# Scthe/cnn-Super-Resolution

Measured on AMD Instinct MI355X. Metric: training tiles/sec (fwd+bwd+update), default SRCNN 33x33, batch 4096/GPU, higher is better.
Workload: dtype f32

## Files before the change

### cnn-super-resolution_amd/csrc/hip/d1x6.hpp

```cpp

constexpr int kD6Mxx = 12, kD6Mx3 = 25;
constexpr int kD6ExWin = 6, kD6ExMid = 3;
constexpr int kD6Grow = 70;

constexpr int kD6Zero = 32;
__device__ __attribute__((aligned(16))) float g_d6_zero[kD6Zero] = {};
constexpr int d6_row_half(bool d3, int h) { return (d3 ? 4 : 8) * h; }
constexpr int d6_zero_half(bool d3, int h) { return d6_row_half(d3, h); }
constexpr int d6_row_quad(bool d3, int k) { return d3 ? 8 * k : 16 * (k >> 1) + 4 * (k & 1); }
constexpr bool d6_zero_row_covers(bool d3) {
  for (int h = 0; h < 2; h++)
    for (int k = 0; k < 4; k++)
      if (d6_zero_half(d3, h) + d6_row_quad(d3, k) + 4 > kD6Zero) return false;
  return true;
}

__device__ __forceinline__ void mma_x6_2(const bf16x8 (&a0)[3], const bf16x8 (&b0)[3], f32x16& c0,
                                         const bf16x8 (&a1)[3], const bf16x8 (&b1)[3], f32x16& c1) {
  using mfma::mma_bf16;
  c0 = mma_bf16(a0[2], b0[0], c0);
  c1 = mma_bf16(a1[2], b1[0], c1);
  c0 = mma_bf16(a0[1], b0[1], c0);
  c1 = mma_bf16(a1[1], b1[1], c1);
  c0 = mma_bf16(a0[0], b0[2], c0);
  c1 = mma_bf16(a1[0], b1[2], c1);
  c0 = mma_bf16(a0[1], b0[0], c0);
  c1 = mma_bf16(a1[1], b1[0], c1);
  c0 = mma_bf16(a0[0], b0[1], c0);
  c1 = mma_bf16(a1[0], b1[1], c1);
  c0 = mma_bf16(a0[0], b0[0], c0);
  c1 = mma_bf16(a1[0], b1[0], c1);
}

__device__ __forceinline__ void d6_split(const float (&v)[8], bf16x8 (&o)[3]) { mfma::split8(v, o); }

template <bool kD3, bool kTr = false>
__global__ __launch_bounds__(256, 1) void d1x6_grad12_kernel(const float* __restrict__ X,
                                                              const float* __restrict__ A1T,
                                                              const float* __restrict__ D2,
                                                              const float* __restrict__ A2,
                                                              const uint32_t* __restrict__ M2,
                                                              const float* __restrict__ W2,
                                                              const float* __restrict__ W3,
                                                              float* __restrict__ slab, Geom g, RunGeom rg,
                                                              D3Geom dg) {
  constexpr int N1 = 64, N2 = 32, F1 = 9, K1 = F1 * F1;
  constexpr int NW1 = K1 * N1, NW2 = N1 * N2, P12 = NW1 + N1 + NW2 + N2;
  extern __shared__ __attribute__((aligned(16))) float smem[];
  static_assert(kD3 || !kTr, "the part images belong to the delta3 form");
  const D6Lds L(g.W, g.H, rg, kD3);
  char* const base = reinterpret_cast<char*>(smem);
  __bf16* const w2i = reinterpret_cast<__bf16*>(base + L.w2);
  uint32_t* const u32 = reinterpret_cast<uint32_t*>(smem);
  uint32_t* const xbuf = u32 + L.xb / 4;
  int* const slots = reinterpret_cast<int*>(base + L.slots);
  int* const runs = reinterpret_cast<int*>(base + L.runs);

  SRCNN_CLOCK_BEGIN();
  const int lane = mfma::lane_id(), wave = mfma::wave_id();
  const int h = lane >> 5, li = lane & 31;
  const int W = g.W, xn = g.W * g.H, npx = g.ow * g.oh, nch = rg.nch;
  const int x0col = 4 * rg.a;

  float xr[kL12Regs];
  auto xload = [&](int smp) {
    const float* src = X + (size_t)smp * xn;
#pragma unroll
    for (int k = 0; k < kL12Regs; k++) {
      const int i = threadIdx.x + 256 * k;
      xr[k] = i < xn ? src[i] : 0.0f;
    }
  };
  if ((int)blockIdx.x < g.batch) xload(blockIdx.x);

  if constexpr (!kTr)
    for (int i = threadIdx.x; i < nch * 32; i += 256) slots[i] = slot_pixel(rg, i >> 5, i & 31);
  for (int k = threadIdx.x; k < nch * 8; k += 256) {
    int iy, ix;
    bool col;
    run_origin(rg, k < rg.nrun ? k : 0, iy, ix, col);
    runs[(k & ~7) + 4 * (k & 1) + 2 * ((k >> 2) & 1) + ((k >> 1) & 1)] =
        col ? ~(L.rdw + 3 * ((ix - x0col) * L.st + iy)) : 3 * (iy * L.rs + ix);
  }
  for (int i = threadIdx.x; i < (2 * L.xbuf + 3) / 4; i += 256) reinterpret_cast<uint4*>(xbuf)[i] = uint4{0u, 0u, 0u, 0u};
  if (threadIdx.x < 32 && (!kD3 || threadIdx.x < kD6Mxx || (threadIdx.x >= 16 && threadIdx.x < kD6Mx3)))
    u32[L.cst / 4 + threadIdx.x] = !kD3 && (threadIdx.x == 0 || threadIdx.x == 6) ? 0x3F803F80u : 0u;
  {
    constexpr int kIt = 2 * 2 * 64 * 8 / 256;
    float v[kIt];
#pragma unroll
    for (int k = 0; k < kIt; k++) {
      const int e = threadIdx.x + 256 * k;
      const int j = e & 7, L_ = (e >> 3) & 63, kk = (e >> 9) & 1, t = e >> 10;
      const int n = kD3 ? crow(8 * kk + j, L_ >> 5) : 16 * kk + 8 * (L_ >> 5) + j;
      v[k] = W2[(32 * t + (L_ & 31)) * N2 + n];
    }
#pragma unroll
    for (int k = 0; k < kIt; k++) {
      const int e = threadIdx.x + 256 * k;
      const int j = e & 7, L_ = (e >> 3) & 63, kk = (e >> 9) & 1, t = e >> 10;
      __bf16 p[3];
      split3(v[k], p[0], p[1], p[2]);
#pragma unroll
      for (int q = 0; q < 3; q++) w2i[((t * 2 + kk) * 3 + q) * 512 + L_ * 8 + j] = p[q];
    }
  }

  uint32_t* const d3u = u32 + L.d3img / 4;
  const int nout3 = dg.w3 * dg.h3;
// ... 21 lines not shown
          b16[2 * (d + L.gw * q) - 1] = b;
        }
      }
    }
  };
  float* const mxx = smem + L.cst / 4 + kD6Mxx;
  float* const mx3 = smem + L.cst / 4 + kD6Mx3;
  auto wave_max = [&](float v) {
#pragma unroll
    for (int o = 32; o > 0; o >>= 1) v = fmaxf(v, __shfl_xor(v, o, 64));
    return v;
  };
  auto put_max = [&](float* slot, float v) {
    v = wave_max(v);
    if (lane == 0) slot[wave] = v;
  };
  auto take_max_reg = [&](float v) {
    return __builtin_bit_cast(float, __builtin_amdgcn_readfirstlane(__builtin_bit_cast(int, v)));
  };
  auto take_max = [&](const float* slot) {
    const float v = fmaxf(fmaxf(slot[0], slot[1]), fmaxf(slot[2], slot[3]));
    return __builtin_bit_cast(float, __builtin_amdgcn_readfirstlane(__builtin_bit_cast(int, v)));
  };
  float m3cur = 0.0f, wnorm = 0.0f;
  int EW = 0, EB = 0, EWmin = 1 << 20, EBmin = 1 << 20;
  if constexpr (kD3) {
    {
      float n2 = 0.0f, n3 = 0.0f;
      for (int n = 0; n < N2; n++) n2 += fabsf(W2[lane * N2 + n]);
      for (int t = 0; t < dg.f3 * dg.f3; t++) n3 += fabsf(W3[t * N2 + li]);
      wnorm = take_max_reg(wave_max(n2)) * take_max_reg(wave_max(n3));
    }
    __bf16* const w3i = reinterpret_cast<__bf16*>(base + L.w3i);
    constexpr int kW3It = 2 * 64 * 8 / 256;
    static_assert(kW3It * 256 * 3 == kD6W3, "the W3 image: 2 k-steps x 3 parts");
    float w3v[kW3It];
#pragma unroll
    for (int k = 0; k < kW3It; k++) {
      const int e = threadIdx.x + 256 * k;
      const int j = e & 7, L_ = (e >> 3) & 63, s_ = e >> 9;
      const D3Pair tp = d3_pair_slot(8 * s_ + 4 * (L_ >> 5) + (j >> 1), dg.f3);
      const int dx = d3_pair_dx(tp, j & 1, dg.f3), n = L_ & 31;
      const bool in = dx >= 0;
      w3v[k] = W3[in ? (tp.dy * dg.f3 + dx) * N2 + n : 0];
      if (!in) w3v[k] = 0.0f;
    }
#pragma unroll
    for (int k = 0; k < kW3It; k++) {
      const int e = threadIdx.x + 256 * k;
      const int j = e & 7, L_ = (e >> 3) & 63, s_ = e >> 9;
      __bf16 p[3];
      split3(w3v[k], p[0], p[1], p[2]);
#pragma unroll
      for (int q = 0; q < 3; q++) w3i[((s_ * 3 + q) * 64 + L_) * 8 + j] = p[q];
    }
    int* const d3tab = reinterpret_cast<int*>(base + L.d3tab);
    for (int i = threadIdx.x; i < nch * 32; i += 256) {
      int iy, ix;
      slot_coord(rg, i >> 5, i & 31, iy, ix);
      d3tab[i] = kTr ? d6_slot_pack(slot_pixel(rg, i >> 5, i & 31), iy * L.gs + ix) : iy * L.gs + ix;
    }
    for (int i = threadIdx.x; i < (3 * L.d3buf + 3) / 4; i += 256)
      reinterpret_cast<uint4*>(d3u)[i] = uint4{0u, 0u, 0u, 0u};
    if ((int)blockIdx.x < g.batch) d3load(blockIdx.x);
    put_max(mx3, fmaxf(fabsf(d3n[0]), fabsf(d3n[1])));
    __syncthreads();
    m3cur = take_max(mx3);
    d3build(0);
    if ((int)blockIdx.x + (int)gridDim.x < g.batch) d3load(blockIdx.x + gridDim.x);
  }

  int offR3[3], offT3[3];
#pragma unroll
  for (int u = 0; u < 3; u++) {
    const int tap = 32 * u + li;
    const int dy = tap < K1 ? tap / F1 : 0, dx = tap < K1 ? tap - dy * F1 : 0;
    offR3[u] = 12 * (dy * L.rs + dx);
    offT3[u] = 12 * (dx * L.st + dy);
  }
  typedef __attribute__((address_space(3))) const uint32_t lds_u32;
  const int lds0 = (int)(uintptr_t)(__attribute__((address_space(3))) char*)base;
  const int spec = li == K1 - 64 ? lds0 + L.cst : li > K1 - 64 ? lds0 + L.cst + 64 : -1;

  f32x16 g1[2][3], g2[2];
#pragma unroll
  for (int t = 0; t < 2; t++) {
    g2[t] = zero16();
#pragma unroll
    for (int u = 0; u < 3; u++) g1[t][u] = zero16();
  }
// ... 179 lines not shown
    } else {
      take_rows();
    }
  }
  if constexpr (kTr) {
    sum_d2(1.0f);
#pragma unroll
    for (int k = 0; k < 2; k++) {
      split_d2(1 + k);
      tr_write(k);
    }
    __builtin_amdgcn_wave_barrier();
    tr_read(0);
    tr_read(1);
  } else {
    stage_d2();
#pragma unroll
    for (int piece = 0; piece < 5; piece++) split_d2(piece);
  }

  for (int it = 0; (int)blockIdx.x + it * (int)gridDim.x < g.batch; it++) {
    const int smp = blockIdx.x + it * gridDim.x;
    uint32_t* const xi = xbuf + (it & 1) * L.xbuf;
    float s1 = 1.0f, sX = 1.0f;
    float m3next = 0.0f;
    if constexpr (kD3) {
      float xm = 0.0f;
#pragma unroll
      for (int k = 0; k < kL12Regs; k++) xm = fmaxf(xm, fabsf(xr[k]));
      float dm = fmaxf(fabsf(d3n[0]), fabsf(d3n[1]));
#pragma unroll
      for (int o = 32; o > 0; o >>= 1) {
        const float tx = __shfl_xor(xm, o, 64), td = __shfl_xor(dm, o, 64);
        xm = fmaxf(xm, tx);
        dm = fmaxf(dm, td);
      }
      if (lane == 0) {
        mxx[wave] = xm;
        mx3[wave] = dm;
      }
      if (smp + (int)gridDim.x < g.batch) d3build((it + 1) - 3 * ((it + 1) / 3));
      __syncthreads();
      const float xmax = take_max(mxx);
      m3next = take_max(mx3);
      const float bound = m3cur * wnorm;
      int e1 = mfma::scale_exp_h(bound), exn = mfma::scale_exp_h(xmax), ex = 0, kb = 0, dW = 0, dB = 0;
      if (exn < mfma::kScaleMin + kD6ExMid) exn = mfma::kScaleMin + kD6ExMid;
      if (bound > 0.0f) {
        int exc = e1 + exn - kD6ExMid - (EWmin + kD6Grow);
        if (exc < e1 - (EBmin + kD6Grow)) exc = e1 - (EBmin + kD6Grow);
        if (exc > 0) e1 = e1 - exc < mfma::kScaleMin ? mfma::kScaleMin : e1 - exc;
        kb = EB - e1;
        if (kb < -14 || kb > 15) {
          dB = e1 - EB;
          EB = e1;
          kb = 0;
        }
        if (xmax > 0.0f) {
          ex = EW - e1;
          if (ex > exn || ex < exn - kD6ExWin) {
            ex = exn - kD6ExMid;
            dW = e1 + ex - EW;
            EW = e1 + ex;
          }
        }
        if (EW < EWmin) EWmin = EW;
        if (EB < EBmin) EBmin = EB;
      } else {
        e1 = 0;
        ex = xmax > 0.0f ? exn - kD6ExMid : 0;
      }
      s1 = mfma::pow2_h(e1);
      sX = mfma::pow2_h(ex);
      if (threadIdx.x == 0) {
        const uint32_t c = (uint32_t)(kb + 15) << 10;
        u32[L.cst / 4 + 3 * (it & 1)] = u32[L.cst / 4 + 3 * (it & 1) + 6] = c | (c << 16);
      }
      while (dW != 0 || dB != 0) {
        const int a = dW < -120 ? -120 : dW > 120 ? 120 : dW, b = dB < -120 ? -120 : dB > 120 ? 120 : dB;
        const float fw = mfma::pow2_h(a), fb = li == K1 - 64 ? mfma::pow2_h(b) : fw;
#pragma unroll
        for (int t = 0; t < 2; t++)
#pragma unroll
          for (int u = 0; u < 3; u++) {
            const float f = u == 2 ? fb : fw;
#pragma unroll
            for (int r = 0; r < 16; r++) g1[t][u][r] *= f;
            __builtin_amdgcn_sched_barrier(0);
          }
        dW -= a;
        dB -= b;
      }
    }
    if constexpr (kD3) {
      uint16_t* const x16 = reinterpret_cast<uint16_t*>(xi);
#pragma unroll
      for (int k = 0; k < kL12Regs; k++) {
        const int i = threadIdx.x + 256 * k;
        if (i < xn) {
          const float xs = xr[k] * sX;
          const _Float16 p0 = (_Float16)xs;
          const _Float16 p[2] = {p0, (_Float16)(xs - (float)p0)};
          const int y = i / W, x = i - y * W, ri = y * L.rs + x;
          const int ti = L.rdw + 3 * ((x - x0col) * L.st + y);
#pragma unroll
          for (int q = 0; q < 2; q++) {
            const uint16_t b = __builtin_bit_cast(uint16_t, p[q]);
            x16[2 * (3 * ri + q)] = b;
            if (ri > 0) x16[2 * (3 * (ri - 1) + q) + 1] = b;
            if (L.tcols && x >= x0col) {
              x16[2 * (ti + q)] = b;
              if (y > 0) x16[2 * (ti - 3 + q) + 1] = b;
            }
          }
        }
// ... 226 lines not shown
            }
            stage_d2();
          }
          if (st == 1) split_d2(0);
          if (st >= 1 && st <= 4) split_d2(st);
        } else if (st < 2) {
          split_d1(1, st);
          if (st == 1) split_d2(0);
        } else {
          split_d2(st - 1);
        }
#pragma unroll
        for (int i = 0; i < (kD3 ? 6 : 12); i++) {
          __builtin_amdgcn_sched_group_barrier(0x008, 1, 0);
          __builtin_amdgcn_sched_group_barrier(0x002, kD3 ? 12 : 6, 0);
          __builtin_amdgcn_sched_group_barrier(0x100, kD3 ? 2 : 1, 0);
        }
        __builtin_amdgcn_sched_barrier(0);
      }
      ki += 4;
      kj = nj;
      kc = nc;
    }
    m3cur = m3next;
  }
  SRCNN_CLOCK_END(g_clk, 2);

  __syncthreads();
  float* const red = smem;
  float* out = slab + (size_t)blockIdx.x * P12;
  float* const stg = smem + 4 * 4 * 16 * 64;
  auto stg_w1 = [&](int row, int ch) -> float& { return stg[row * N1 + (ch ^ ((row & 15) << 2))]; };
  auto tile_ref = [&](int k) -> f32x16& { return k < 6 ? g1[k / 3][k % 3] : g2[k - 6]; };
#pragma unroll
  for (int rd = 0; rd < 2; rd++) {
#pragma unroll
    for (int k = 0; k < 4; k++) {
      const f32x16& a = tile_ref(4 * rd + k);
#pragma unroll
      for (int r = 0; r < 16; r++) red[((k * 4 + wave) * 16 + r) * 64 + lane] = a[r];
    }
    __syncthreads();
#pragma unroll
    for (int k = 0; k < 4; k++) {
      if (wave != k) continue;
      const int tile = 4 * rd + k;
      f32x16 sum;
// ... 62 lines not shown
```

### cnn-super-resolution_amd/csrc/hip/fused_layout.hpp

```cpp
#include "runs.hpp"
#include "d6tr.hpp"

constexpr int kLdsMax = 160 * 1024;
constexpr int kLdsHalf = kLdsMax / 2;

struct Geom {
  int W, H;
  int ow, oh;
  int batch;
};

constexpr int kXsMax = 1536;
constexpr int kL12S = 57;
constexpr int kL12Rows = 40;
constexpr int kL12Tile = kL12S * (kL12Rows + 1);
constexpr int kL12Regs = (kXsMax + 255) / 256;
constexpr int kL12Grid = 512, kL3RGrid = 512;

struct L3Geom {
  int W, H;
  int w2, h2;
  int w3, h3;
  int batch;
};
// ... 100 lines not shown
}

constexpr int kH6W1 = kX6KS * 2 * 2 * 512;
constexpr int kH6W2 = 4 * 2 * 512;
constexpr int kH6Cst = 128 + 32 + 32 + 12;
struct H6Lds {
  int rs, r, xs, a2sc, bytes;
  __host__ __device__ H6Lds(int w, int h) {
    const int a4 = (4 * ((w - 8) / 4)) % 32;
    r = (kH6W1 + kH6W2) * 2 + kH6Cst * 4;
    rs = X6Lds(w, h).pad ? 2 * w + ((a4 - 2 * w) % 32 + 32) % 32 : 2 * w;
    xs = r + (rs * h + 1) * 4;
    a2sc = (xs + w * h * 4 + 15) & ~15;
    bytes = a2sc + 4 * kX6Sc * 4;
  }
};

constexpr int kD6W2 = 2 * 2 * 3 * 512;
constexpr int kD6W3 = 2 * 3 * 512;
constexpr int kD6Sc = 32 * 36;

struct D3Geom {
  int w3, h3, f3;
};

struct D6Lds {
  int st;
  int tcols;
  int rs;
  int rdw;
  int tdw;
  int xbuf;
  int gw, gs, gh, d3buf;
  int w2, xb, sc, slots, runs, cst, w3i, d3tab, d3img, bytes;
  int tr;
  __host__ __device__ D6Lds(int w, int h, const RunGeom& rg, bool d3 = false) {
    st = 4 * rg.cr + 9;
    if (st < h + 1) st = h + 1;
    tcols = rg.b ? rg.b + 8 : 0;
    rs = w + ((9 - w) % 64 + 64) % 64;
    rdw = 3 * (rs * h + 1);
    tdw = 3 * tcols * st;
    xbuf = rdw + tdw;
    w2 = 0;
    xb = kD6W2 * 2;
    sc = xb + 2 * xbuf * 4;
// ... 45 lines not shown
```

### cnn-super-resolution_amd/csrc/hip/fused_plan.hpp

```cpp
#include "net.hpp"

template <typename F>
static int with_net(const srcnn_net* net, F&& f) {
  return first_net(net, f, Net<64, 32, 9, 5>{},
                   Net<32, 16, 9, 5>{},
                   Net<64, 32, 9, 3>{}, Net<32, 16, 9, 3>{});
}

static int grid_for_batch(uint32_t batch, int cap) { return (int)std::min<uint32_t>(batch, cap); }

struct StepPlan {
  int ow, oh, w3, h3;
  bool x6, l3r, l3_fused, d3mode, kD1c;
  bool d1tr;
  int d1c_parts;
  RunGeom rg;
  int g12, g3, gd;
  size_t lds12, lds3, ldsd;
  size_t s12, s3, ssq;
  size_t bytes;
  size_t m2_off;
  int a1_layout;
  const char *k12, *k3, *kd1;
};

template <typename NetT>
static bool plan_step(uint32_t w, uint32_t h, uint32_t batch, int arith, StepPlan* out) {
  constexpr int N2 = NetT::N2, F1 = NetT::F1, F3 = NetT::F3;
  StepPlan& p = *out = {};
  const int ow = p.ow = w - F1 + 1, oh = p.oh = h - F1 + 1;
  const int w3 = p.w3 = ow - F3 + 1, h3 = p.h3 = oh - F3 + 1;
  if ((int)(w * h) > kXsMax || (int)w > kL12S || (int)h > kL12Rows || w3 <= 0 || h3 <= 0) return false;
  p.l3r = N2 == 32 && l3r_fits<F3>(ow, oh, w3, h3);
  p.lds3 = p.l3r ? L3RLds<F3>(ow, oh).bytes() : l3_lds_bytes<N2, F3>(ow, oh);
  p.l3_fused =
      p.l3r || (p.lds3 <= (size_t)kLdsMax && w3 * h3 <= kL3MaxOut &&
                ((ow * oh + 15) / 16 + kL3Threads / 64 - 1) / (kL3Threads / 64) <= L3Lds<N2, F3>::kUnitsPerWave);
  p.g12 = grid_for_batch(batch, kL12Grid);
  p.x6 = NetT::kDefault12 && arith == 0 && l12x6_fits(w, h) && d1x6_fits(w, h);
  p.a1_layout = p.x6 ? kA1Runs : kA1Blocked;
  p.rg = run_geom(ow, oh);
  const int b3 = (int)batch;
  p.g3 = p.l3r ? std::min(kL3RGrid, std::max(std::min(b3, 256), (b3 + 1) / 2)) : grid_for_batch(batch, 256);
  p.kD1c = NetT::kDefault12 && d1c_fits(w, h);
  const int nch1 = (ow * oh + 31) / 32;
  p.d1c_parts = p.kD1c ? std::max(1, std::min({4, nch1, kD1cGrid / (int)std::max<uint32_t>(batch, 1)})) : 1;
  while (p.d1c_parts > 1 && (p.d1c_parts - 1) * ((nch1 + p.d1c_parts - 1) / p.d1c_parts) >= nch1)
    p.d1c_parts--;
  p.m2_off = ((size_t)batch * w3 * h3 + 63) & ~(size_t)63;
  p.d3mode = p.x6 && p.l3r && F3 <= 5 && d1x6_fits(w, h, true) && l3r_d3_fits<F3>(ow, oh) &&
             p.m2_off + (size_t)batch * ow * oh <= (size_t)batch * ow * oh * N2;
  const int gd6 = grid_for_batch(batch, 256);
  const int gdf = p.kD1c ? (int)std::min<size_t>((size_t)batch * p.d1c_parts, kD1cGrid) : grid_for_batch(batch, 512);
  p.gd = p.x6 ? gd6 : gdf;
  p.lds12 = p.x6 ? H6Lds(w, h).bytes : 0;
  const D6Lds ld6(w, h, p.rg, p.d3mode);
  p.ldsd = p.x6 ? ld6.bytes : p.kD1c ? d1c_lds_bytes(w, h) : 0;
  p.d1tr = p.x6 && p.d3mode && ld6.tr;
  p.k12 = p.x6 ? "l12x6_fwd" : "l12_fwd";
  p.k3 = !p.l3_fused ? "l3_op_level" : !p.l3r ? "l3_delta" : p.d3mode ? "l3r_d3" : "l3r_delta";
  p.kd1 = p.x6 ? (p.d1tr ? "d1x6_d3" : p.d3mode ? "d1x6_d3_sc" : "d1x6_grad12") : p.kD1c ? "d1c_grad12" : "d1_grad12";
  p.s12 = (size_t)std::max(gd6, gdf) * NetT::P12;
  p.s3 = (size_t)p.g3 * NetT::P3;
  p.ssq = p.g3;
  if (!p.l3_fused) {
    p.s3 = fast::grad_workspace_bytes(N2, 1, F3, w3, h3, batch) / sizeof(float);
    if (p.s3 == 0) return false;
    p.s3 = std::max<size_t>(p.s3, reduce_blocks((size_t)batch * w3 * h3) + 1);
    p.ssq = 0;
  }
  p.bytes = (p.s12 + p.s3 + p.ssq) * sizeof(float);
  return true;
}
```

### cnn-super-resolution_amd/csrc/hip/l12x6.hpp

```cpp
using mfma::bf16x8;
using mfma::f16x8;
using mfma::mma_x3_h;
using mfma::mma_x6;
using mfma::relu1;
using mfma::split3;
using mfma::split8;
using mfma::split8_h;
using mfma::split8_pk;
using mfma::u32x4;

template <bool kLazy>
__global__ __launch_bounds__(256, 2) void l12x6_fwd_kernel(const float* __restrict__ X,
                                                            const float* __restrict__ W1,
                                                            const float* __restrict__ B1,
                                                            const float* __restrict__ W2,
                                                            const float* __restrict__ B2,
                                                            float* __restrict__ A1,
                                                            float* __restrict__ A2, Geom g, RunGeom rg,
                                                            LazyUpdate lz) {
  constexpr int N1 = 64, N2 = 32, F1 = 9, NT1 = 2;
  extern __shared__ __attribute__((aligned(16))) float smem[];
  const H6Lds L(g.W, g.H);
  _Float16* const w1i = reinterpret_cast<_Float16*>(smem);
  _Float16* const w2i = w1i + kH6W1;
  float* const a88s = reinterpret_cast<float*>(w2i + kH6W2);
  float* const b2i = a88s + 128;
  float* const b2s = b2i + 32;
  float* const wmx = b2s + 32;
  float* const w2mx = wmx + 4;
  float* const xmx = w2mx + 4;
  uint32_t* const rimg = reinterpret_cast<uint32_t*>(reinterpret_cast<char*>(smem) + L.r);
  float* const xs = reinterpret_cast<float*>(reinterpret_cast<char*>(smem) + L.xs);
  const int rs = L.rs;
  float* const a2sc = reinterpret_cast<float*>(reinterpret_cast<char*>(smem) + L.a2sc);

  SRCNN_CLOCK_BEGIN();
  const int lane = mfma::lane_id(), wave = mfma::wave_id();
  const int h = lane >> 5, li = lane & 31;
  const int W = g.W, xn = g.W * g.H;
  const int npx = g.ow * g.oh, nch = rg.nch;

  float xr[kL12Regs];
// ... 144 lines not shown
    if (pok) {
      if (k < 16 * NT1) {
        const int t = k >> 4, r = k & 15;
        __builtin_nontemporal_store(pa1[t][r], pa1p + (32 * t + crow(r, h)) * 32);
      } else {
        const int q = k - 16 * NT1;
        if (ppx[q] >= 0) {
          f32x4 v_;
#pragma unroll
          for (int e = 0; e < 4; e++) v_[e] = pa2[4 * q + e];
          *reinterpret_cast<f32x4*>(pa2p + (size_t)ppx[q] * N2 + 4 * (lane & 7)) = v_;
        }
      }
    }
  };

  const uint16_t* const wl1 = reinterpret_cast<const uint16_t*>(w1i) + lane * 8;
  const uint16_t* const wl2 = reinterpret_cast<const uint16_t*>(w2i) + lane * 8;
  auto w1op = [&](int s, int t, f16x8 (&a)[2]) {
#pragma unroll
    for (int q = 0; q < 2; q++) a[q] = *reinterpret_cast<const f16x8*>(wl1 + ((s * 2 + t) * 2 + q) * 512);
  };

  for (int sample = blockIdx.x; sample < g.batch; sample += gridDim.x) {
    {
      float xm = 0.0f;
#pragma unroll
      for (int k = 0; k < kL12Regs; k++) xm = fmaxf(xm, fabsf(xr[k]));
      xm = wave_max(xm);
      if (lane == 0) xmx[wave] = xm;
    }
    __syncthreads();
    const int ex = mfma::scale_exp_h(max4(xmx));
    const float sx = mfma::pow2_h(ex);
    const int eu = -(ew + ex), eu1 = eu > 127 ? 127 : eu;
    const float un1 = mfma::pow2_h(eu1), un2 = mfma::pow2_h(eu - eu1);
    const int ea = mfma::scale_exp_h(max4(xmx) * wnorm + b1max);
    const float sa = mfma::pow2_h(ea);
    const int ev = -(ea + ew2), ev1 = ev > 127 ? 127 : ev;
    const float vn1 = mfma::pow2_h(ev1), vn2 = mfma::pow2_h(ev - ev1);
    if (threadIdx.x < 32) b2s[threadIdx.x] = b2i[threadIdx.x] * sa;
    {
      uint16_t* const r16 = reinterpret_cast<uint16_t*>(rimg);
#pragma unroll
      for (int k = 0; k < kL12Regs; k++) {
        const int i = threadIdx.x + 256 * k;
        if (i < xn) {
          const float xv = xr[k] * sx;
          xs[i] = xv;
          const int y = i / W, x = i - y * W, d = y * rs + x;
          const _Float16 q0 = (_Float16)xv, q1 = (_Float16)(xv - (float)q0);
          const uint16_t b0 = __builtin_bit_cast(uint16_t, q0), b1 = __builtin_bit_cast(uint16_t, q1);
          r16[2 * d] = b0;
          r16[2 * (d + W)] = b1;
          if (x > 0) {
            r16[2 * d - 1] = b0;
// ... 105 lines not shown
          f32x4 v_;
#pragma unroll
          for (int e = 0; e < 4; e++) v_[e] = relu1(acc2[4 * m + e]);
          *reinterpret_cast<f32x4*>(sc + li * 32 + 4 * ((2 * m + h) ^ (li & 7))) = v_;
        }
        if (h == 0) scp[li] = pv ? iy * g.ow + ix : -1;
        __builtin_amdgcn_wave_barrier();
#pragma unroll
        for (int q = 0; q < 4; q++) {
          const int p_ = 8 * q + (lane >> 3);
          const f32x4 v_ = *reinterpret_cast<const f32x4*>(sc + p_ * 32 + 4 * ((lane & 7) ^ (p_ & 7)));
#pragma unroll
          for (int e = 0; e < 4; e++) pa2[4 * q + e] = v_[e];
          ppx[q] = scp[8 * q + (lane >> 3)];
        }
      }
      pok = true;
      pa1p = A1 + ((size_t)sample * nch + c) * (32 * N1) + li;
      pa2p = A2 + (size_t)sample * npx * N2;
    }
  }
#pragma unroll
  for (int k = 0; k < NST; k++) store_prev(k);
  SRCNN_CLOCK_END(g_clk, 0);
}
```

### cnn-super-resolution_amd/csrc/hip/l3r.hpp

```cpp

template <int F3>
__host__ __device__ constexpr int l3r_tap(int s, int lg) {
  return s < F3 ? (lg < F3 ? lg * F3 + s : -1)
                : (F3 == 5 && s < 7 && 4 * (s - 5) + lg < 5 ? 20 + 4 * (s - 5) + lg : -1);
}
template <int F3>
constexpr int l3r_kt() { return F3 == 5 ? 7 : F3; }

__device__ __forceinline__ f32x4 ld_a2(const float* p) {
  return __builtin_nontemporal_load(reinterpret_cast<const f32x4*>(p));
}
__device__ __forceinline__ void st_d2(float* p, f32x4 v) {
  __builtin_nontemporal_store(v, reinterpret_cast<f32x4*>(p));
}

template <int F3, bool kD3Out>
__global__ __launch_bounds__(kL3RThreads, 4) void l3r_delta_kernel(
    const float* __restrict__ A2, const float* __restrict__ T, const float* __restrict__ W3,
    const float* __restrict__ B3, float* __restrict__ D2, float* __restrict__ slab3,
    float* __restrict__ sq_slab, float* __restrict__ A3out, uint32_t* __restrict__ M2, L3Geom g) {
  constexpr int N2 = 32;
  constexpr int K3 = F3 * F3;
  constexpr int TT = (K3 + 15) / 16;
  constexpr int NT = 2;
  constexpr int KT = l3r_kt<F3>();
  constexpr int NW3 = K3 * N2;
  constexpr int nwaves = kL3RThreads / 64;
  static_assert(K3 <= 32, "taps must fit two 16-wide MFMA tiles");
  SRCNN_CLOCK_BEGIN();
  extern __shared__ __attribute__((aligned(16))) float smem[];
  const int npx2 = g.w2 * g.h2;
  const L3RLds<F3> L(g.w2, g.h2);
  const int d3off = L.d3off;
  float* qs = smem;
  float* w3s = smem + L.qreg;
  float* wds = w3s + L.w3img;
  float* d3g = wds + L.wdimg + 4;
  float* red = smem;

  const int tid = threadIdx.x;
  const int lane = mfma::lane_id(), wave = mfma::wave_id();
  const int lq = lane & 15, lg = lane >> 4;
  const int pad = (g.W - g.w3) / 2;
// ... 37 lines not shown
    agb[t] = goff[t] + 4 * lg + 16 * wave;
    asm volatile("" : "+v"(agb[t]));
  }

  const int wqo = lq * kL3RW3S + 4 * lg;
  float* scw = smem + wave * (32 * kL3RScS);
  static_assert(kL3RW3S == kL3RWdS && kL3RW3S == kL3RScS, "shared lane base");
  const int sco_w = 4 * lg * kL3RScS + lq;
  const int srw = lq * kL3RScS + 4 * lg;
  const int srr = (lq & 7) * kL3RScS + 4 * (lg + 4 * (lq >> 3));

  f32x4 gacc[TT][NT];
#pragma unroll
  for (int t3 = 0; t3 < TT; t3++)
#pragma unroll
    for (int t = 0; t < NT; t++) gacc[t3][t] = mfma::zero4();
  f32x16 g3x = zero16();
  uint32_t* const d3p = reinterpret_cast<uint32_t*>(smem + 8 * 32 * kL3RScS);

  const int li32 = lane & 31, h32 = lane >> 5;
  const int g3b = d3off - tap_off(li32 < K3 ? li32 : 0) + 16 * wave + 8 * h32;
  const int g3s = li32 * kL3RScS + 8 * h32;
  float gb3 = 0.0f, sq = 0.0f;

  f32x4 a2r[kL3RUnits][2];
  const bool lo8 = lq < 8;
#define SRCNN_L3R_LOAD(J, SAMPLE)                                                       \
  do {                                                                                  \
              \
              \
    int l_ = lane;                                                                      \
    asm volatile("" : "+v"(l_));                                                        \
    const int lo_ = ((l_ & 7) * N2 + 4 * ((l_ >> 4) + 4 * ((l_ >> 3) & 1)));            \
    const int pa_ = 16 * (wave + nwaves * (J)) + (l_ & 7);                              \
    const float* b_ = A2 + (size_t)(SAMPLE)*npx2 * N2;                                  \
    const unsigned w_ = 16 * (wave + nwaves * (J)) * N2 + lo_;                          \
    const unsigned oa_ = pa_ < npx2 ? w_ : lo_;    \
    const unsigned ob_ = pa_ + 8 < npx2 ? w_ + 8 * N2 : lo_;                            \
    a2r[J][0] = ld_a2(b_ + oa_);                                                        \
    a2r[J][1] = ld_a2(b_ + ob_);                                                        \
  } while (0)
#define SRCNN_L3R_SWAP(J)                                                               \
  do {                                                                                  \
    _Pragma("unroll") for (int i_ = 0; i_ < 4; i_++) {                                  \
      const float a_ = a2r[J][0][i_], b_ = a2r[J][1][i_];                               \
      const float r_ = __builtin_bit_cast(float, __builtin_amdgcn_mov_dpp(               \
// ... 89 lines not shown
        }
      }
    }
    asm volatile("s_waitcnt lgkmcnt(0)" ::: "memory");
    __builtin_amdgcn_s_barrier();
    asm volatile("" ::: "memory");

#pragma unroll
    for (int k = 0; k < kL3RTPF; k++) {
      const int t = tid + k * kL3RThreads;
      if (t < nout) {
        const int y = t / g.w3, x = t - y * g.w3;
        const float* qrow = qs + (y * g.w2 + x) * K3;
        float acc = 0.0f;
#pragma unroll
        for (int dy = 0; dy < F3; dy++)
#pragma unroll
          for (int dx = 0; dx < F3; dx++) acc += qrow[(dy * g.w2 + dx) * K3 + dy * F3 + dx];
        const float a3 = acc + b3;
        A3out[(size_t)smp * nout + t] = a3;
        const float diff = a3 - tcur[k];
        const float d3 = diff * (a3 > 0.0f ? 1.0f : 0.0f);
        d3g[y * g.w2 + x + d3off] = d3;
        if constexpr (kD3Out) D2[(size_t)smp * nout + t] = d3;
        gb3 += d3;
        sq += diff * diff;
      }
    }
    asm volatile("s_waitcnt lgkmcnt(0)" ::: "memory");
    __builtin_amdgcn_s_barrier();
    asm volatile("" ::: "memory");
    if constexpr (kD3Out) {
      for (int gi = tid - 4; gi < L.nd3 - 5; gi += kL3RThreads) {
        uint32_t pp[3];
        mfma::split_pair(d3g[gi], d3g[gi + 1], pp);
#pragma unroll
        for (int q = 0; q < 3; q++) d3p[q * L.nd3 + gi + 4] = pp[q];
      }
      asm volatile("s_waitcnt lgkmcnt(0)" ::: "memory");
      __builtin_amdgcn_s_barrier();
      asm volatile("" ::: "memory");
    }

    float* d2s = D2 + (kD3Out ? 0 : ((size_t)smp * npx2 + 16 * wave) * N2);
#pragma unroll
    for (int j = 0; j < kL3RUnits; j++) {
      __builtin_amdgcn_sched_barrier(0);
// ... 122 lines not shown
#pragma unroll
  for (int t3 = 0; t3 < TT; t3++)
#pragma unroll
    for (int t = 0; t < NT; t++)
#pragma unroll
      for (int i = 0; i < 4; i++) {
        const int idx = (t3 * NT + t) * 4 + i;
        red[wave * kRed + idx * 64 + lane] = kD3Out ? g3x[idx] : gacc[t3][t][i];
      }
  __syncthreads();
  float* out = slab3 + (size_t)blockIdx.x * (NW3 + 1);
  for (int i = tid; i < kRed; i += kL3RThreads) {
    float v = red[i];
    for (int w = 1; w < nwaves; w++) v += red[w * kRed + i];
    const int k = i >> 8, r = (i >> 6) & 3, l = i & 63;
    const int t3 = k / NT, t = k - t3 * NT;
    const int tap = kD3Out ? crow(i >> 6, l >> 5) : 16 * t3 + 4 * (l >> 4) + r;
    const int n = kD3Out ? (l & 31) : 16 * t + (l & 15);
    if (tap < K3) out[tap * N2 + n] = v;
  }
  for (int off = 32; off > 0; off >>= 1) {
    gb3 += __shfl_down(gb3, off, 64);
    sq += __shfl_down(sq, off, 64);
  }
  __syncthreads();
  if (lane == 0) {
    red[2 * wave] = gb3;
    red[2 * wave + 1] = sq;
  }
  __syncthreads();
  if (tid == 0) {
    float tb = 0.f, ts = 0.f;
    for (int w = 0; w < nwaves; w++) {
      tb += red[2 * w];
      ts += red[2 * w + 1];
    }
    out[NW3] = tb;
    sq_slab[blockIdx.x] = ts;
  }
}
```

### cnn-super-resolution_amd/csrc/hip/train_fused.hip

```cpp
#include <algorithm>
#include <cstdlib>
#include <cstring>
#include <string>
#include <type_traits>

#include "common.hpp"
#include "lds_dma.hpp"
#include "mfma.hpp"
#include "ops.hpp"
#include "split.hpp"

namespace srcnn {
namespace fused {

using mfma::crow;
using mfma::f32x16;
using mfma::f32x4;
using mfma::mma;
using mfma::zero16;

__device__ unsigned long long g_clk[3][kClockBlocks][2];

constexpr int kNtMask = 9;

// ... 29 lines not shown
  SRCNN_LAUNCH_TRY();
  return SRCNN_OK;
}

static thread_local const float* t_a1_region = nullptr;
static thread_local int t_a1_layout = -1;

template <typename NetT>
static int run(const StepPlan& p, const srcnn_net* net, uint32_t w, uint32_t h, uint32_t batch,
               const StepBuffers& b, hipStream_t s, const SlabUpdate* up, const LazyUpdate* lz) {
  constexpr int N1 = NetT::N1, N2 = NetT::N2, F1 = NetT::F1, F3 = NetT::F3;
  if (b.slab_bytes < p.bytes)
    return fail(SRCNN_ERR_WORKSPACE, "fused train step: slab workspace %zu B < %zu B", b.slab_bytes, p.bytes);
  float* slab12 = b.slab;
  float* slab3 = slab12 + p.s12;
  float* sqs = slab3 + p.s3;
  const float *X = b.X, *T = b.T;
  float *grads = b.grads, *A1 = b.A1, *A2 = b.A2, *D2 = b.D2, *A3 = b.A3;
  const bool lazy = lz && lz->batch > 0.0f;
  const LazyUpdate lu = lazy ? *lz : LazyUpdate{};
  const auto P = split_params(lazy ? lz->Po : b.params, net);
  const int ow = p.ow, oh = p.oh, w3 = p.w3, h3 = p.h3;
  const Geom g{(int)w, (int)h, ow, oh, (int)batch};
  {
    SRCNN_PROFILE("l12_fwd_mfma", s);
    kernels_note(lazy ? (std::string(p.k12) + "_lazy").c_str() : p.k12);
    note_a1_layout(A1, p.a1_layout);
    const dim3 grid(p.g12), blk(256);
    const auto k6 = lazy ? l12x6_fwd_kernel<true> : l12x6_fwd_kernel<false>;
    const auto k = lazy ? l12_fwd_kernel<N1, N2, F1, true> : l12_fwd_kernel<N1, N2, F1>;
    if (int rc = p.x6 ? launch(k6, grid, blk, p.lds12, s, X, P.W1, P.B1, P.W2, P.B2, A1, A2, g, p.rg, lu)
                      : launch(k, grid, blk, 0, s, X, P.W1, P.B1, P.W2, P.B2, A1, A2, g, lu))
      return rc;
  }
  if (lz && !p.l3_fused)
    SRCNN_HIP_TRY(hipMemsetAsync(grads + NetT::P12, 0, NetT::P3 * sizeof(float), s));
  const L3Geom lg{(int)w, (int)h, ow, oh, w3, h3, (int)batch};
  uint32_t* M2 = p.d3mode ? reinterpret_cast<uint32_t*>(D2) + p.m2_off : nullptr;
  kernels_note(p.k3);
  if (p.l3_fused) {
    SRCNN_PROFILE("l3_delta_fused", s);
    const dim3 grid(p.g3);
    const auto kr = p.d3mode ? l3r_delta_kernel<F3, true> : l3r_delta_kernel<F3, false>;
    if (int rc = p.l3r ? launch(kr, grid, dim3(kL3RThreads), p.lds3, s, A2, T, P.W3, P.B3, D2, slab3, sqs, A3, M2, lg)
                       : launch(l3_delta_kernel<N2, F3>, grid, dim3(kL3Threads), p.lds3, s, A2, T, P.W3, P.B3, D2, slab3, sqs, A3, lg))
      return rc;
  } else {
    const int rf = fast::try_conv_fwd(A2, A3, P.W3, P.B3, ow, oh, N2, 1, F3, 0, batch, s);
    if (rf != 1) return rf < 0 ? rf : fail(SRCNN_ERR_INVALID, "fused step: no layer-3 kernel for %dx%d", ow, oh);
    if (b.sq_err)
      if (int rc = reduce(2, A3, T, (size_t)batch * w3 * h3, w, h, w3, h3, b.sq_err, 1, slab3,
                          p.s3 * sizeof(float), s))
        return rc;
    if (int rc = generic::last_delta(T, A3, b.D3, w, h, w3, h3, batch, s)) return rc;
    const int rd = fast::try_conv_delta(b.D3, A2, D2, P.W3, F3, N2, 1, ow, oh, batch, s);
    if (rd != 1) return rd < 0 ? rd : fail(SRCNN_ERR_INVALID, "fused step: no delta2 kernel for %dx%d", ow, oh);
    const int rg = fast::try_conv_grad_acc(A2, b.D3, grads + NetT::P12, grads + NetT::P12 + NetT::P3 - 1, N2, 1,
                                           F3, w3, h3, batch, slab3, p.s3 * sizeof(float), s);
    if (rg != 1) return rg < 0 ? rg : fail(SRCNN_ERR_INVALID, "fused step: no gW3 kernel for %dx%d", ow, oh);
  }
  {
    SRCNN_PROFILE("delta1_grad12_fused", s);
    kernels_note(p.kd1);
    const dim3 grid(p.gd), blk(256);
    const D3Geom dg{w3, h3, F3};
    const auto k6 = p.d1tr ? d1x6_grad12_kernel<true, true> : p.d3mode ? d1x6_grad12_kernel<true> : d1x6_grad12_kernel<false>;
    if (int rc = p.x6 ? launch(k6, grid, blk, p.ldsd, s, X, A1, D2, A2, M2, P.W2, P.W3, slab12, g, p.rg, dg)
                 : p.kD1c ? launch(d1c_grad12_kernel<9>, grid, dim3(256 * kD1cTeams), p.ldsd, s, X, A1, D2, P.W2, slab12, g,
                                   d1c_xs_floats(h), p.d1c_parts)
                          : launch(d1_grad12_kernel<N1, N2, F1>, grid, blk, 0, s, X, A1, D2, P.W2, slab12, g))
      return rc;
  }
  SRCNN_PROFILE("slab_reduce", s);
  const bool update = up && p.l3_fused;
  kernels_note(update ? "slab_reduce_update" : "slab_reduce");
  const SlabSeg segs[3] = {{slab12, grads, p.gd, NetT::P12, 0},
                           {slab3, grads + NetT::P12, p.g3, NetT::P3, 0},
                           {sqs, b.sq_err, p.g3, 1, 0}};
  SlabUpdate u{};
  if (update) {
    u = *up;
    u.nseg = 2;
  }
  const int assign = lz ? (p.l3_fused ? 2 : 1) : 0;
  if (int rc = p.l3_fused ? reduce_slabs(segs, b.sq_err ? 3 : 2, s, &u, assign) : reduce_slabs(segs, 1, s, nullptr, assign))
    return rc;
  return update ? 2 : 1;
}

bool train_plan(const srcnn_net* net, uint32_t w, uint32_t h, uint32_t batch, StepNeed* need) {
// ... 74 lines not shown
```

Baseline: 6.484 million.

## Use batch-global input and delta maxima for fixed per-kernel scaling exponents

The forward layer-1/2 kernel and the layer-3 delta kernel now write per-block maxima of |x| and |delta3| to scratch space. The delta1/grad12 kernel reduces these once at start to pick a single scaling exponent for the whole launch. This removes the per-sample wave reductions, the __syncthreads, the exponent bookkeeping and the accumulator rescale loops from the inner sample loop. The cost is extra scratch writes and reads, plus coarser per-sample scaling that may lose precision for samples with small magnitudes.

```diff
diff --git a/cnn-super-resolution_amd/csrc/hip/d1x6.hpp b/cnn-super-resolution_amd/csrc/hip/d1x6.hpp
--- a/cnn-super-resolution_amd/csrc/hip/d1x6.hpp
+++ b/cnn-super-resolution_amd/csrc/hip/d1x6.hpp
@@ -1,7 +1,5 @@
 
 constexpr int kD6Mxx = 12, kD6Mx3 = 25;
-constexpr int kD6ExWin = 6, kD6ExMid = 3;
-constexpr int kD6Grow = 70;
 
 constexpr int kD6Zero = 32;
 __device__ __attribute__((aligned(16))) float g_d6_zero[kD6Zero] = {};
@@ -40,6 +38,8 @@
                                                               const float* __restrict__ D2,
                                                               const float* __restrict__ A2,
                                                               const uint32_t* __restrict__ M2,
+                                                              const float* __restrict__ xmaxs,
+                                                              const float* __restrict__ d3maxs, D6MaxGeom mg,
                                                               const float* __restrict__ W2,
                                                               const float* __restrict__ W3,
                                                               float* __restrict__ slab, Geom g, RunGeom rg,
@@ -72,6 +72,17 @@
     }
   };
   if ((int)blockIdx.x < g.batch) xload(blockIdx.x);
+  float lmx = 0.0f, lm3 = 0.0f;
+  if constexpr (kD3) {
+    static_assert(kL12Grid <= 512 && kL3RGrid <= 512, "two slots per thread");
+#pragma unroll
+    for (int k = 0; k < 2; k++) {
+      const int i = threadIdx.x + 256 * k;
+      const float a = i < mg.n12 ? xmaxs[i] : 0.0f, b = i < mg.n3 ? d3maxs[i] : 0.0f;
+      lmx = fmaxf(lmx, a);
+      lm3 = fmaxf(lm3, b);
+    }
+  }
 
   if constexpr (!kTr)
     for (int i = threadIdx.x; i < nch * 32; i += 256) slots[i] = slot_pixel(rg, i >> 5, i & 31);
@@ -83,8 +94,10 @@
         col ? ~(L.rdw + 3 * ((ix - x0col) * L.st + iy)) : 3 * (iy * L.rs + ix);
   }
   for (int i = threadIdx.x; i < (2 * L.xbuf + 3) / 4; i += 256) reinterpret_cast<uint4*>(xbuf)[i] = uint4{0u, 0u, 0u, 0u};
-  if (threadIdx.x < 32 && (!kD3 || threadIdx.x < kD6Mxx || (threadIdx.x >= 16 && threadIdx.x < kD6Mx3)))
-    u32[L.cst / 4 + threadIdx.x] = !kD3 && (threadIdx.x == 0 || threadIdx.x == 6) ? 0x3F803F80u : 0u;
+  if (threadIdx.x < 32 && (!kD3 || threadIdx.x < kD6Mxx || (threadIdx.x >= 16 && threadIdx.x < kD6Mx3))) {
+    const bool one = threadIdx.x == 0 || threadIdx.x == 6 || (kD3 && (threadIdx.x == 3 || threadIdx.x == 9));
+    u32[L.cst / 4 + threadIdx.x] = one ? (kD3 ? 0x3C003C00u : 0x3F803F80u) : 0u;
+  }
   {
     constexpr int kIt = 2 * 2 * 64 * 8 / 256;
     float v[kIt];
@@ -152,8 +165,9 @@
     const float v = fmaxf(fmaxf(slot[0], slot[1]), fmaxf(slot[2], slot[3]));
     return __builtin_bit_cast(float, __builtin_amdgcn_readfirstlane(__builtin_bit_cast(int, v)));
   };
-  float m3cur = 0.0f, wnorm = 0.0f;
-  int EW = 0, EB = 0, EWmin = 1 << 20, EBmin = 1 << 20;
+  float wnorm = 0.0f;
+  int EW = 0, EB = 0;
+  float s1 = 1.0f, sX = 1.0f;
   if constexpr (kD3) {
     {
       float n2 = 0.0f, n3 = 0.0f;
@@ -193,9 +207,17 @@
     for (int i = threadIdx.x; i < (3 * L.d3buf + 3) / 4; i += 256)
       reinterpret_cast<uint4*>(d3u)[i] = uint4{0u, 0u, 0u, 0u};
     if ((int)blockIdx.x < g.batch) d3load(blockIdx.x);
-    put_max(mx3, fmaxf(fabsf(d3n[0]), fabsf(d3n[1])));
+    put_max(mxx, lmx);
+    put_max(mx3, lm3);
     __syncthreads();
-    m3cur = take_max(mx3);
+    {
+      const float xmax = take_max(mxx), bound = take_max(mx3) * wnorm;
+      const int e1 = bound > 0.0f ? mfma::scale_exp_h(bound) : 0, ex = xmax > 0.0f ? mfma::scale_exp_h(xmax) : 0;
+      EW = e1 + ex;
+      EB = e1;
+      s1 = mfma::pow2_h(e1);
+      sX = mfma::pow2_h(ex);
+    }
     d3build(0);
     if ((int)blockIdx.x + (int)gridDim.x < g.batch) d3load(blockIdx.x + gridDim.x);
   }
@@ -421,75 +443,8 @@
   for (int it = 0; (int)blockIdx.x + it * (int)gridDim.x < g.batch; it++) {
     const int smp = blockIdx.x + it * gridDim.x;
     uint32_t* const xi = xbuf + (it & 1) * L.xbuf;
-    float s1 = 1.0f, sX = 1.0f;
-    float m3next = 0.0f;
     if constexpr (kD3) {
-      float xm = 0.0f;
-#pragma unroll
-      for (int k = 0; k < kL12Regs; k++) xm = fmaxf(xm, fabsf(xr[k]));
-      float dm = fmaxf(fabsf(d3n[0]), fabsf(d3n[1]));
-#pragma unroll
-      for (int o = 32; o > 0; o >>= 1) {
-        const float tx = __shfl_xor(xm, o, 64), td = __shfl_xor(dm, o, 64);
-        xm = fmaxf(xm, tx);
-        dm = fmaxf(dm, td);
-      }
-      if (lane == 0) {
-        mxx[wave] = xm;
-        mx3[wave] = dm;
-      }
       if (smp + (int)gridDim.x < g.batch) d3build((it + 1) - 3 * ((it + 1) / 3));
-      __syncthreads();
-      const float xmax = take_max(mxx);
-      m3next = take_max(mx3);
-      const float bound = m3cur * wnorm;
-      int e1 = mfma::scale_exp_h(bound), exn = mfma::scale_exp_h(xmax), ex = 0, kb = 0, dW = 0, dB = 0;
-      if (exn < mfma::kScaleMin + kD6ExMid) exn = mfma::kScaleMin + kD6ExMid;
-      if (bound > 0.0f) {
-        int exc = e1 + exn - kD6ExMid - (EWmin + kD6Grow);
-        if (exc < e1 - (EBmin + kD6Grow)) exc = e1 - (EBmin + kD6Grow);
-        if (exc > 0) e1 = e1 - exc < mfma::kScaleMin ? mfma::kScaleMin : e1 - exc;
-        kb = EB - e1;
-        if (kb < -14 || kb > 15) {
-          dB = e1 - EB;
-          EB = e1;
-          kb = 0;
-        }
-        if (xmax > 0.0f) {
-          ex = EW - e1;
-          if (ex > exn || ex < exn - kD6ExWin) {
-            ex = exn - kD6ExMid;
-            dW = e1 + ex - EW;
-            EW = e1 + ex;
-          }
-        }
-        if (EW < EWmin) EWmin = EW;
-        if (EB < EBmin) EBmin = EB;
-      } else {
-        e1 = 0;
-        ex = xmax > 0.0f ? exn - kD6ExMid : 0;
-      }
-      s1 = mfma::pow2_h(e1);
-      sX = mfma::pow2_h(ex);
-      if (threadIdx.x == 0) {
-        const uint32_t c = (uint32_t)(kb + 15) << 10;
-        u32[L.cst / 4 + 3 * (it & 1)] = u32[L.cst / 4 + 3 * (it & 1) + 6] = c | (c << 16);
-      }
-      while (dW != 0 || dB != 0) {
-        const int a = dW < -120 ? -120 : dW > 120 ? 120 : dW, b = dB < -120 ? -120 : dB > 120 ? 120 : dB;
-        const float fw = mfma::pow2_h(a), fb = li == K1 - 64 ? mfma::pow2_h(b) : fw;
-#pragma unroll
-        for (int t = 0; t < 2; t++)
-#pragma unroll
-          for (int u = 0; u < 3; u++) {
-            const float f = u == 2 ? fb : fw;
-#pragma unroll
-            for (int r = 0; r < 16; r++) g1[t][u][r] *= f;
-            __builtin_amdgcn_sched_barrier(0);
-          }
-        dW -= a;
-        dB -= b;
-      }
     }
     if constexpr (kD3) {
       uint16_t* const x16 = reinterpret_cast<uint16_t*>(xi);
@@ -762,7 +717,6 @@
       kj = nj;
       kc = nc;
     }
-    m3cur = m3next;
   }
   SRCNN_CLOCK_END(g_clk, 2);
 
diff --git a/cnn-super-resolution_amd/csrc/hip/fused_layout.hpp b/cnn-super-resolution_amd/csrc/hip/fused_layout.hpp
--- a/cnn-super-resolution_amd/csrc/hip/fused_layout.hpp
+++ b/cnn-super-resolution_amd/csrc/hip/fused_layout.hpp
@@ -146,6 +146,9 @@
 
 struct D3Geom {
   int w3, h3, f3;
+};
+struct D6MaxGeom {
+  int n12, n3;
 };
 
 struct D6Lds {
diff --git a/cnn-super-resolution_amd/csrc/hip/fused_plan.hpp b/cnn-super-resolution_amd/csrc/hip/fused_plan.hpp
--- a/cnn-super-resolution_amd/csrc/hip/fused_plan.hpp
+++ b/cnn-super-resolution_amd/csrc/hip/fused_plan.hpp
@@ -20,6 +20,7 @@
   size_t s12, s3, ssq;
   size_t bytes;
   size_t m2_off;
+  size_t mx_off, d3mx_off;
   int a1_layout;
   const char *k12, *k3, *kd1;
 };
@@ -48,8 +49,11 @@
   while (p.d1c_parts > 1 && (p.d1c_parts - 1) * ((nch1 + p.d1c_parts - 1) / p.d1c_parts) >= nch1)
     p.d1c_parts--;
   p.m2_off = ((size_t)batch * w3 * h3 + 63) & ~(size_t)63;
+  p.mx_off = (p.m2_off + (size_t)batch * ow * oh + 63) & ~(size_t)63;
+  p.d3mx_off = (p.mx_off + p.g12 + 63) & ~(size_t)63;
   p.d3mode = p.x6 && p.l3r && F3 <= 5 && d1x6_fits(w, h, true) && l3r_d3_fits<F3>(ow, oh) &&
-             p.m2_off + (size_t)batch * ow * oh <= (size_t)batch * ow * oh * N2;
+             p.m2_off + (size_t)batch * ow * oh <= (size_t)batch * ow * oh * N2 &&
+             p.d3mx_off + kL3RGrid <= (size_t)batch * ow * oh * N2;
   const int gd6 = grid_for_batch(batch, 256);
   const int gdf = p.kD1c ? (int)std::min<size_t>((size_t)batch * p.d1c_parts, kD1cGrid) : grid_for_batch(batch, 512);
   p.gd = p.x6 ? gd6 : gdf;
diff --git a/cnn-super-resolution_amd/csrc/hip/l12x6.hpp b/cnn-super-resolution_amd/csrc/hip/l12x6.hpp
--- a/cnn-super-resolution_amd/csrc/hip/l12x6.hpp
+++ b/cnn-super-resolution_amd/csrc/hip/l12x6.hpp
@@ -17,7 +17,7 @@
                                                             const float* __restrict__ B2,
                                                             float* __restrict__ A1,
                                                             float* __restrict__ A2, Geom g, RunGeom rg,
-                                                            LazyUpdate lz) {
+                                                            LazyUpdate lz, float* __restrict__ xmax) {
   constexpr int N1 = 64, N2 = 32, F1 = 9, NT1 = 2;
   extern __shared__ __attribute__((aligned(16))) float smem[];
   const H6Lds L(g.W, g.H);
@@ -208,6 +208,7 @@
     for (int q = 0; q < 2; q++) a[q] = *reinterpret_cast<const f16x8*>(wl1 + ((s * 2 + t) * 2 + q) * 512);
   };
 
+  float xrun = 0.0f;
   for (int sample = blockIdx.x; sample < g.batch; sample += gridDim.x) {
     {
       float xm = 0.0f;
@@ -218,6 +219,7 @@
     }
     __syncthreads();
     const int ex = mfma::scale_exp_h(max4(xmx));
+    xrun = fmaxf(xrun, max4(xmx));
     const float sx = mfma::pow2_h(ex);
     const int eu = -(ew + ex), eu1 = eu > 127 ? 127 : eu;
     const float un1 = mfma::pow2_h(eu1), un2 = mfma::pow2_h(eu - eu1);
@@ -369,5 +371,6 @@
   }
 #pragma unroll
   for (int k = 0; k < NST; k++) store_prev(k);
+  if (xmax != nullptr && threadIdx.x == 0 && (int)blockIdx.x < g.batch) xmax[blockIdx.x] = xrun;
   SRCNN_CLOCK_END(g_clk, 0);
 }
diff --git a/cnn-super-resolution_amd/csrc/hip/l3r.hpp b/cnn-super-resolution_amd/csrc/hip/l3r.hpp
--- a/cnn-super-resolution_amd/csrc/hip/l3r.hpp
+++ b/cnn-super-resolution_amd/csrc/hip/l3r.hpp
@@ -18,7 +18,8 @@
 __global__ __launch_bounds__(kL3RThreads, 4) void l3r_delta_kernel(
     const float* __restrict__ A2, const float* __restrict__ T, const float* __restrict__ W3,
     const float* __restrict__ B3, float* __restrict__ D2, float* __restrict__ slab3,
-    float* __restrict__ sq_slab, float* __restrict__ A3out, uint32_t* __restrict__ M2, L3Geom g) {
+    float* __restrict__ sq_slab, float* __restrict__ A3out, uint32_t* __restrict__ M2,
+    float* __restrict__ d3max, L3Geom g) {
   constexpr int N2 = 32;
   constexpr int K3 = F3 * F3;
   constexpr int TT = (K3 + 15) / 16;
@@ -102,6 +103,7 @@
   const int g3b = d3off - tap_off(li32 < K3 ? li32 : 0) + 16 * wave + 8 * h32;
   const int g3s = li32 * kL3RScS + 8 * h32;
   float gb3 = 0.0f, sq = 0.0f;
+  float dmx = 0.0f;
 
   f32x4 a2r[kL3RUnits][2];
   const bool lo8 = lq < 8;
@@ -237,7 +239,10 @@
         const float diff = a3 - tcur[k];
         const float d3 = diff * (a3 > 0.0f ? 1.0f : 0.0f);
         d3g[y * g.w2 + x + d3off] = d3;
-        if constexpr (kD3Out) D2[(size_t)smp * nout + t] = d3;
+        if constexpr (kD3Out) {
+          D2[(size_t)smp * nout + t] = d3;
+          dmx = fmaxf(dmx, fabsf(d3));
+        }
         gb3 += d3;
         sq += diff * diff;
       }
@@ -406,11 +411,13 @@
   for (int off = 32; off > 0; off >>= 1) {
     gb3 += __shfl_down(gb3, off, 64);
     sq += __shfl_down(sq, off, 64);
+    if constexpr (kD3Out) dmx = fmaxf(dmx, __shfl_down(dmx, off, 64));
   }
   __syncthreads();
   if (lane == 0) {
     red[2 * wave] = gb3;
     red[2 * wave + 1] = sq;
+    if constexpr (kD3Out) red[2 * nwaves + wave] = dmx;
   }
   __syncthreads();
   if (tid == 0) {
@@ -421,5 +428,10 @@
     }
     out[NW3] = tb;
     sq_slab[blockIdx.x] = ts;
+    if constexpr (kD3Out) {
+      float tm = 0.f;
+      for (int w = 0; w < nwaves; w++) tm = fmaxf(tm, red[2 * nwaves + w]);
+      if ((int)blockIdx.x < g.batch) d3max[blockIdx.x] = tm;
+    }
   }
 }
diff --git a/cnn-super-resolution_amd/csrc/hip/train_fused.hip b/cnn-super-resolution_amd/csrc/hip/train_fused.hip
--- a/cnn-super-resolution_amd/csrc/hip/train_fused.hip
+++ b/cnn-super-resolution_amd/csrc/hip/train_fused.hip
@@ -75,6 +75,8 @@
   const auto P = split_params(lazy ? lz->Po : b.params, net);
   const int ow = p.ow, oh = p.oh, w3 = p.w3, h3 = p.h3;
   const Geom g{(int)w, (int)h, ow, oh, (int)batch};
+  float* const xmax = p.d3mode ? D2 + p.mx_off : nullptr;
+  float* const d3max = p.d3mode ? D2 + p.d3mx_off : nullptr;
   {
     SRCNN_PROFILE("l12_fwd_mfma", s);
     kernels_note(lazy ? (std::string(p.k12) + "_lazy").c_str() : p.k12);
@@ -82,7 +84,7 @@
     const dim3 grid(p.g12), blk(256);
     const auto k6 = lazy ? l12x6_fwd_kernel<true> : l12x6_fwd_kernel<false>;
     const auto k = lazy ? l12_fwd_kernel<N1, N2, F1, true> : l12_fwd_kernel<N1, N2, F1>;
-    if (int rc = p.x6 ? launch(k6, grid, blk, p.lds12, s, X, P.W1, P.B1, P.W2, P.B2, A1, A2, g, p.rg, lu)
+    if (int rc = p.x6 ? launch(k6, grid, blk, p.lds12, s, X, P.W1, P.B1, P.W2, P.B2, A1, A2, g, p.rg, lu, xmax)
                       : launch(k, grid, blk, 0, s, X, P.W1, P.B1, P.W2, P.B2, A1, A2, g, lu))
       return rc;
   }
@@ -95,7 +97,7 @@
     SRCNN_PROFILE("l3_delta_fused", s);
     const dim3 grid(p.g3);
     const auto kr = p.d3mode ? l3r_delta_kernel<F3, true> : l3r_delta_kernel<F3, false>;
-    if (int rc = p.l3r ? launch(kr, grid, dim3(kL3RThreads), p.lds3, s, A2, T, P.W3, P.B3, D2, slab3, sqs, A3, M2, lg)
+    if (int rc = p.l3r ? launch(kr, grid, dim3(kL3RThreads), p.lds3, s, A2, T, P.W3, P.B3, D2, slab3, sqs, A3, M2, d3max, lg)
                        : launch(l3_delta_kernel<N2, F3>, grid, dim3(kL3Threads), p.lds3, s, A2, T, P.W3, P.B3, D2, slab3, sqs, A3, lg))
       return rc;
   } else {
@@ -117,8 +119,9 @@
     kernels_note(p.kd1);
     const dim3 grid(p.gd), blk(256);
     const D3Geom dg{w3, h3, F3};
+    const D6MaxGeom mg{p.g12, p.g3};
     const auto k6 = p.d1tr ? d1x6_grad12_kernel<true, true> : p.d3mode ? d1x6_grad12_kernel<true> : d1x6_grad12_kernel<false>;
-    if (int rc = p.x6 ? launch(k6, grid, blk, p.ldsd, s, X, A1, D2, A2, M2, P.W2, P.W3, slab12, g, p.rg, dg)
+    if (int rc = p.x6 ? launch(k6, grid, blk, p.ldsd, s, X, A1, D2, A2, M2, xmax, d3max, mg, P.W2, P.W3, slab12, g, p.rg, dg)
                  : p.kD1c ? launch(d1c_grad12_kernel<9>, grid, dim3(256 * kD1cTeams), p.ldsd, s, X, A1, D2, P.W2, slab12, g,
                                    d1c_xs_floats(h), p.d1c_parts)
                           : launch(d1_grad12_kernel<N1, N2, F1>, grid, blk, 0, s, X, A1, D2, P.W2, slab12, g))
```

After: 7.006 million, median of 6. +8.0%, better.
